# Rose-STL-Lab/spherical-dyffusion

Hardware: AMD Instinct MI355X
Metric: forecast-steps/sec (180x360, 63ch), 25-member ensemble DYffusion sampling, whole job (higher is better)
Workload: dtype f32 tensors; every GEMM-class kernel (1x1 convs, fused MLP, Legendre analysis/synthesis, dhconv) as 3-pass split-f16 MFMA with f32 accumulation; FFT / norms / pointwise in f32 (statistics f64)

## Files before the change

### include/sdy_amd.h

```cpp
#ifndef SDY_AMD_H
#define SDY_AMD_H

#include <stddef.h>
#include <stdint.h>

#ifdef __cplusplus
extern "C" {
#endif
#pragma GCC visibility push(default)

#define SDY_OK 0
#define SDY_ERR_ARG (-1)
#define SDY_ERR_UNSUPPORTED (-2)
#define SDY_ERR_ALIGN (-3)
#define SDY_ERR_WORKSPACE (-4)
#define SDY_ERR_NAME (-5)
#define SDY_ERR_SHAPE (-6)
#define SDY_ERR_STATE (-7)

#define SDY_GRID_EQUIANGULAR 0
#define SDY_GRID_LEGENDRE_GAUSS 1

int sdy_version(void);
const char* sdy_error_string(int code);
// ... 3 lines not shown

typedef struct sdy_sht_plan sdy_sht_plan;

int sdy_sht_tables_host(int nlat, int nlon, int lmax, int mmax, int grid, double* pct, double* w, double* theta);

int sdy_sht_plan_create(int nlat, int nlon, int lmax, int mmax, int grid, sdy_sht_plan** out);
int sdy_sht_plan_create_ex(int nlat, int nlon, int lmax, int mmax, int grid, int gemm_mode, sdy_sht_plan** out);
void sdy_sht_plan_destroy(sdy_sht_plan* plan);
int sdy_sht_plan_dims(const sdy_sht_plan* plan, int dims[6]);
int sdy_sht_plan_kernels(const sdy_sht_plan* plan, int out[2]);
size_t sdy_sht_workspace_floats(const sdy_sht_plan* plan, int B, int C);

int sdy_sht_forward(const sdy_sht_plan* plan, const float* x, float* out_c64, int B, int C, float* ws,
                    size_t ws_floats, void* stream);
int sdy_sht_inverse(const sdy_sht_plan* plan, const float* in_c64, float* y, int B, int C, float* ws,
                    size_t ws_floats, void* stream);

int sdy_rfft_lon(const sdy_sht_plan* plan, const float* x, const float* a, const float* d, float* xn_out,
                 float* Xf, int B, int C, void* stream);
int sdy_legendre_fwd(const sdy_sht_plan* plan, const float* Xf, float* Cs, int B, int C, void* stream);
int sdy_legendre_inv(const sdy_sht_plan* plan, const float* Cs, float* Yf, int B, int C, void* stream);
int sdy_irfft_lon(const sdy_sht_plan* plan, const float* Yf, const float* bias, float* y, int B, int C,
                  void* stream);
int sdy_irfft_lon_act(const sdy_sht_plan* plan, const float* Yf, const float* bias, float* zt, long zt_bstride, double* part,
                      int B, int C, void* stream);
int sdy_instnorm_from_partials(const double* part, int K, int B, int C, int HW, const float* gamma, const float* beta,
                               float eps, float* a, float* d, void* stream);
int sdy_gelu_stats(const float* y, long y_bstride, float* out, long out_bstride, int out_tiled, double* stats, int B, int C,
                   int HW, void* stream);
int sdy_affine_copy_stats(const float* x, long x_bstride, const float* a, const float* d, float* out, long out_bstride,
                          double* stats, int C, int HW, const unsigned char* rows, int n_rows, int src_row0, void* stream);

int sdy_dhconv_pack_weight(const float* w_host, int Ci, int Co, int L, float* w_packed_dev, void* stream);
int sdy_dhconv(const float* Cs_in, const float* w_packed, float* Cs_out, int L, int mtr, int B, int Ci, int Co,
               void* stream);
size_t sdy_dhconv_h3_pack_bytes(int Ci, int Co, int L);
int sdy_dhconv_h3_pack_weight(const float* w_host, int Ci, int Co, int L, void* packed_dev, float* scale);
int sdy_dhconv_h3(const float* Cs_in, const void* packed, float scale, float* Cs_out, int L, int mtr, int B, int Ci,
                  int Co, void* stream);

int sdy_dhconv_frag_supported(int Ci, int Co);
size_t sdy_dhconv_frag_pack_bytes(int L);
int sdy_dhconv_frag_pack(const float* w_host, int L, void* packed_dev, float* scale);
int sdy_dhconv_frag(const float* Cs_in, const void* packed, float scale, float* Cs_out, int L, int mtr, int B,
                    void* stream);

// ... 437 lines not shown
```

### spherical-dyffusion_amd/_lib.py

```python
from __future__ import annotations

import ctypes as C
import os

_HERE = os.path.dirname(os.path.abspath(__file__))
LIB_PATH = os.environ.get("SDY_AMD_LIB") or os.path.join(_HERE, "libsdy_amd.so")

SDY_GRID = {"equiangular": 0, "legendre-gauss": 1}


class SdyError(RuntimeError):
    pass


class SdyConvArgs(C.Structure):
    _fields_ = [
        ("x", C.c_void_p), ("x_bstride", C.c_long),
        ("wt", C.c_void_p), ("ldw", C.c_int),
        ("out", C.c_void_p), ("out_bstride", C.c_long),
        ("B", C.c_int), ("Cin", C.c_int), ("Cout", C.c_int), ("HW", C.c_int),
        ("pa", C.c_void_p), ("pd", C.c_void_p),
        ("bias", C.c_void_p),
        ("add", C.c_void_p), ("add_bstride", C.c_long),
        ("add_mode", C.c_int),
# ... 319 lines not shown
               SdyMemberSumArgs, SdyMemberStatsArgs, SdySpectrumArgs, SdyVariabilityArgs, SdyVariabilityMapsArgs,
               SdyVariabilityStatsArgs, SdyRegionSeriesArgs, SdyRankHistArgs)

SIGNATURES = {
    "sdy_version": (C.c_int, []),
    "sdy_error_string": (C.c_char_p, [C.c_int]),
    "sdy_abi_check": (C.c_int, [C.POINTER(C.c_size_t), C.c_int]),
    "sdy_abi_sizes": (C.c_int, [C.POINTER(C.c_size_t), C.c_int]),
    "sdy_sht_tables_host": (C.c_int, [C.c_int, C.c_int, C.c_int, C.c_int, C.c_int, C.c_void_p, C.c_void_p, C.c_void_p]),
    "sdy_sht_plan_create": (C.c_int, [C.c_int, C.c_int, C.c_int, C.c_int, C.c_int, C.POINTER(C.c_void_p)]),
    "sdy_sht_plan_create_ex": (C.c_int, [C.c_int, C.c_int, C.c_int, C.c_int, C.c_int, C.c_int, C.POINTER(C.c_void_p)]),
    "sdy_sht_plan_destroy": (None, [C.c_void_p]),
    "sdy_sht_plan_dims": (C.c_int, [C.c_void_p, C.POINTER(C.c_int * 6)]),
    "sdy_sht_plan_kernels": (C.c_int, [C.c_void_p, C.POINTER(C.c_int * 2)]),
    "sdy_sht_workspace_floats": (C.c_size_t, [C.c_void_p, C.c_int, C.c_int]),
    "sdy_sht_forward": (C.c_int, [C.c_void_p, C.c_void_p, C.c_void_p, C.c_int, C.c_int, C.c_void_p, C.c_size_t, C.c_void_p]),
    "sdy_sht_inverse": (C.c_int, [C.c_void_p, C.c_void_p, C.c_void_p, C.c_int, C.c_int, C.c_void_p, C.c_size_t, C.c_void_p]),
    "sdy_rfft_lon": (C.c_int, [C.c_void_p, C.c_void_p, C.c_void_p, C.c_void_p, C.c_void_p, C.c_void_p, C.c_int, C.c_int, C.c_void_p]),
    "sdy_legendre_fwd": (C.c_int, [C.c_void_p, C.c_void_p, C.c_void_p, C.c_int, C.c_int, C.c_void_p]),
    "sdy_legendre_inv": (C.c_int, [C.c_void_p, C.c_void_p, C.c_void_p, C.c_int, C.c_int, C.c_void_p]),
    "sdy_irfft_lon": (C.c_int, [C.c_void_p, C.c_void_p, C.c_void_p, C.c_void_p, C.c_int, C.c_int, C.c_void_p]),
    "sdy_irfft_lon_act": (C.c_int, [C.c_void_p, C.c_void_p, C.c_void_p, C.c_void_p, C.c_long, C.c_void_p, C.c_int, C.c_int,
                                    C.c_void_p]),
    "sdy_instnorm_from_partials": (C.c_int, [C.c_void_p, C.c_int, C.c_int, C.c_int, C.c_int, C.c_void_p, C.c_void_p, C.c_float,
                                             C.c_void_p, C.c_void_p, C.c_void_p]),
    "sdy_gelu_stats": (C.c_int, [C.c_void_p, C.c_long, C.c_void_p, C.c_long, C.c_int, C.c_void_p, C.c_int, C.c_int, C.c_int,
                                 C.c_void_p]),
    "sdy_affine_copy_stats": (C.c_int, [C.c_void_p, C.c_long, C.c_void_p, C.c_void_p, C.c_void_p, C.c_long, C.c_void_p, C.c_int,
                                        C.c_int, C.c_void_p, C.c_int, C.c_int, C.c_void_p]),
    "sdy_dhconv_pack_weight": (C.c_int, [C.c_void_p, C.c_int, C.c_int, C.c_int, C.c_void_p, C.c_void_p]),
    "sdy_dhconv": (C.c_int, [C.c_void_p, C.c_void_p, C.c_void_p, C.c_int, C.c_int, C.c_int, C.c_int, C.c_int, C.c_void_p]),
    "sdy_dhconv_h3_pack_bytes": (C.c_size_t, [C.c_int, C.c_int, C.c_int]),
    "sdy_dhconv_h3_pack_weight": (C.c_int, [C.c_void_p, C.c_int, C.c_int, C.c_int, C.c_void_p, C.POINTER(C.c_float)]),
    "sdy_dhconv_h3": (C.c_int, [C.c_void_p, C.c_void_p, C.c_float, C.c_void_p, C.c_int, C.c_int, C.c_int, C.c_int, C.c_int,
                                C.c_void_p]),
    "sdy_dhconv_frag_supported": (C.c_int, [C.c_int, C.c_int]),
    "sdy_dhconv_frag_pack_bytes": (C.c_size_t, [C.c_int]),
    "sdy_dhconv_frag_pack": (C.c_int, [C.c_void_p, C.c_int, C.c_void_p, C.POINTER(C.c_float)]),
    "sdy_dhconv_frag": (C.c_int, [C.c_void_p, C.c_void_p, C.c_float, C.c_void_p, C.c_int, C.c_int, C.c_int, C.c_void_p]),
    "sdy_instnorm_coeffs": (C.c_int, [C.c_void_p, C.c_int, C.c_int, C.c_int, C.c_void_p, C.c_void_p, C.c_void_p, C.c_long,
                                      C.c_float, C.c_void_p, C.c_void_p, C.c_void_p]),
    "sdy_conv1x1": (C.c_int, [C.POINTER(SdyConvArgs), C.c_void_p]),
    "sdy_ensemble_metrics": (C.c_int, [C.c_void_p, C.c_void_p, C.c_void_p, C.c_int, C.c_long, C.c_int, C.c_int, C.c_void_p,
                                       C.c_void_p]),
    "sdy_instnorm_from_stats": (C.c_int, [C.c_void_p, C.c_int, C.c_int, C.c_int, C.c_void_p, C.c_void_p, C.c_void_p,
                                          C.c_long, C.c_float, C.c_void_p, C.c_void_p, C.c_void_p]),
# ... 155 lines not shown
```

### spherical-dyffusion_amd/csrc/capi.hip

```cpp
#include <cmath>
#include <cstdio>
#include <cstdlib>
#include <cstring>
#include <mutex>
#include <string>
#include <vector>

#include "common.h"
#include "fft.h"
#include "pointwise.h"

static inline int round_up(int v, int m) { return (v + m - 1) / m * m; }
static inline size_t round_up_sz(size_t v, size_t m) { return (v + m - 1) / m * m; }

template <class F>
static float h3_pack_host(std::vector<_Float16>& buf, int nb, int rows, int K, int rows_pad, int Kpad, F value) {
  float mx = 0.f;
  for (int b = 0; b < nb; ++b)
    for (int r = 0; r < rows; ++r)
      for (int k = 0; k < K; ++k) mx = std::fmax(mx, std::fabs(value(b, r, k)));
  const float s = sdy_h3_scale(mx);
  const size_t plane = (size_t)nb * rows_pad * Kpad;
  buf.assign(2 * plane, (_Float16)0.0f);
  for (int b = 0; b < nb; ++b)
// ... 449 lines not shown

extern "C" int sdy_affine_copy_stats(const float* x, long x_bstride, const float* a, const float* d, float* out,
                                     long out_bstride, double* stats, int C, int HW, const unsigned char* rows, int n_rows,
                                     int src_row0, void* stream) {
  if (!x || !out || !rows || (a == nullptr) != (d == nullptr) || C <= 0 || HW <= 0 || n_rows <= 0 || n_rows > SDY_MAP_MAX ||
      x_bstride < 0 || out_bstride < 0)
    return SDY_ERR_ARG;
  if ((HW & 3) || (x_bstride & 3) || (out_bstride & 3) || !fft_aligned16(x) || !fft_aligned16(out) || !fft_aligned16(stats))
    return SDY_ERR_ALIGN;
  return sdy_affine_copy_stats_launch(x, x_bstride, a, d, out, out_bstride, stats, C, HW, rows, n_rows, (hipStream_t)stream,
                                      src_row0 >= 0 ? src_row0 : -1);
}

extern "C" int sdy_irfft_lon_act(const sdy_sht_plan* p, const float* Yf, const float* bias, float* zt, long zt_bstride,
                                 double* part, int B, int C, void* stream) {
  if (!p || !Yf || !zt || !part || B <= 0 || C <= 0 || zt_bstride < 0) return SDY_ERR_ARG;
  if (C % 4 != 0 || (zt_bstride & 3) || !fft_aligned16(Yf) || !fft_aligned16(zt) || !fft_aligned16(part)) return SDY_ERR_ALIGN;
  if (!(p->fft.fft360 && p->fft.n == 180) || C % 16 != 0) return SDY_ERR_UNSUPPORTED;
  if (!tiled_stride_ok(zt_bstride, C, p->nlat * p->nlon)) return SDY_ERR_ARG;
  return sdy_fft360_launch_inv(p->fft, Yf, bias, nullptr, B, C, p->nlat, p->mtr, 0, nullptr, (hipStream_t)stream, zt, zt_bstride,
                               part);
}

static inline int h3_mpad(int Cout) { return Cout > 128 ? round_up(Cout, 256) : 128; }
static inline int h3_kpad(int Cin) { return round_up(Cin, 64); }

extern "C" size_t sdy_h3_pack_bytes(int Cout, int Cin) {
  if (Cout <= 0 || Cin <= 0) return 0;
  return (size_t)2 * h3_mpad(Cout) * h3_kpad(Cin) * sizeof(_Float16);
}

extern "C" int sdy_h3_pack_weight(const float* w, int Cout, int Cin, void* packed_dev, float* scale) {
  if (!w || !packed_dev || !scale || Cout <= 0 || Cin <= 0) return SDY_ERR_ARG;
  std::vector<_Float16> buf;
  *scale = h3_pack_host(buf, 1, Cout, Cin, h3_mpad(Cout), h3_kpad(Cin),
                        [&](int, int o, int i) { return w[(size_t)o * Cin + i]; });
  SDY_HIP_TRY(hipMemcpy(packed_dev, buf.data(), buf.size() * sizeof(_Float16), hipMemcpyHostToDevice));
  return SDY_OK;
}

extern "C" int sdy_conv1x1(const sdy_conv_args* a, void* stream) {
  if (!a || !a->x || (!a->wt && !a->w_h3 && !a->w_frag) || !a->out) return SDY_ERR_ARG;
  if (a->B <= 0 || a->Cin <= 0 || a->Cout <= 0 || a->HW <= 0) return SDY_ERR_ARG;
  if (!a->w_h3 && a->ldw < a->Cout) return SDY_ERR_ARG;
  if ((a->pa == nullptr) != (a->pd == nullptr)) return SDY_ERR_ARG;
  if (a->add_mode != 0 && !a->add) return SDY_ERR_ARG;
// ... 962 lines not shown
```

### spherical-dyffusion_amd/csrc/fft.h

```cpp
#pragma once
#include <hip/hip_runtime.h>

struct SdyFftDesc {
  int n;
  int S;
  int nstages;
  int radices[10];
  const float* tw;
  const float* pw;
  int guard_f16;
  int fft360;
};


int sdy_fft_launch_fwd(const SdyFftDesc& f, const float* x, const float* a, const float* d, float* xn_out, float* Xf,
                       int B, int C, int K, int mtr, int ilv, const int* mcut, hipStream_t stream,
                       const unsigned char* x_rows = nullptr, int x_mod = 0);
int sdy_fft_launch_inv(const SdyFftDesc& f, const float* Yf, const float* bias, float* y, int B, int C, int K, int mtr,
                       int ilv, const int* mcut, hipStream_t stream);

int sdy_fft360_launch_fwd(const SdyFftDesc& f, const float* x, const float* a, const float* d, float* xn_out, float* Xf,
                          int B, int C, int K, int mtr, int ilv, const int* mcut, hipStream_t stream,
                          const unsigned char* x_rows = nullptr, int x_mod = 0);
int sdy_fft360_launch_inv(const SdyFftDesc& f, const float* Yf, const float* bias, float* y, int B, int C, int K,
                          int mtr, int ilv, const int* mcut, hipStream_t stream, float* zt = nullptr, long zt_bs = 0,
                          double* part = nullptr);
```

### spherical-dyffusion_amd/csrc/fft360.hip

```cpp
#include "common.h"
#include "fft.h"

namespace {

typedef float c2 __attribute__((ext_vector_type(2)));

constexpr int NH = 180;
constexpr int NLON = 360;
constexpr int ROWS = 16;
constexpr int NT = 256;
constexpr int P = 200;
constexpr int Q4 = NLON / 4;
constexpr int MIT = 3;
#ifndef SDY_FFT_MINB_F
#define SDY_FFT_MINB_F 4
#endif
#ifndef SDY_FFT_MINB_I
#define SDY_FFT_MINB_I 4
#endif
#ifndef SDY_FFT_KPW
#define SDY_FFT_KPW 1
#endif
constexpr int MINB_F = SDY_FFT_MINB_F, MINB_I = SDY_FFT_MINB_I;

template <int SG>
__device__ __forceinline__ c2 mul_i(c2 a) {
  return SG > 0 ? c2{-a.y, a.x} : c2{a.y, -a.x};
}
__device__ __forceinline__ c2 cmul(c2 a, c2 w) { return a.xx * w + a.yy * c2{-w.y, w.x}; }
__device__ __forceinline__ c2 cmul_conj(c2 a, c2 w) { return a.xx * c2{w.x, -w.y} + a.yy * c2{w.y, w.x}; }

template <int SG>
__device__ __forceinline__ void dft3(c2& v0, c2& v1, c2& v2) {
  const float sn = 0.86602540378443864676f;
  const c2 a = v1 + v2, b = v1 - v2;
  const c2 m = v0 - 0.5f * a;
  const c2 t = mul_i<SG>(sn * b);
  v0 = v0 + a;
  v1 = m + t;
  v2 = m - t;
}
template <int SG>
__device__ __forceinline__ void dft4(c2& v0, c2& v1, c2& v2, c2& v3) {
  const c2 t0 = v0 + v2, t1 = v0 - v2, t2 = v1 + v3, t3 = mul_i<SG>(v1 - v3);
  v0 = t0 + t2;
  v1 = t1 + t3;
// ... 84 lines not shown
    for (int k2 = 0; k2 < 15; ++k2) dst[12 * k2] = u[pfa_slot<3, 5>(k2)];
    if (NYQ_COPY && L.t == 0) dst[NH] = u[pfa_slot<3, 5>(0)];
  }
  __builtin_amdgcn_wave_barrier();
}
template <int SG>
__device__ __forceinline__ void pass_a_tail(const Lane& L, c2* v, const c2* TW) {
  pfa<3, 4, SG>(v);
  c2* dst = L.row + L.t;
  const c2* tw = TW + L.t;
  dst[0] = v[pfa_slot<3, 4>(0)];
#pragma unroll
  for (int k1 = 1; k1 < 12; ++k1) {
    const c2 y = v[pfa_slot<3, 4>(k1)];
    dst[15 * k1] = SG < 0 ? cmul(y, tw[16 * k1]) : cmul_conj(y, tw[16 * k1]);
  }
}

constexpr int TAIL = Q4 - 64;

#ifndef SDY_FFT_GROUP
#define SDY_FFT_GROUP 4
#endif
struct WgId {
  int x, y, z;
};
__device__ __forceinline__ WgId wg_id(int nx, int ny) {
  const unsigned total = gridDim.x, L = blockIdx.x;
  const unsigned xcd = L % 8u, slot = L / 8u;
  const unsigned id = xcd * (total / 8u) + min(xcd, total % 8u) + slot;
  WgId w;
#if SDY_FFT_GROUP > 0
  if (nx % SDY_FFT_GROUP == 0) {
    const unsigned G = SDY_FFT_GROUP;
    w.x = (int)(G * ((id / (G * ny)) % ((unsigned)nx / G)) + id % G);
    w.y = (int)((id / G) % (unsigned)ny);
    w.z = (int)(id / ((unsigned)nx * ny));
    return w;
  }
#endif
  w.x = id % nx;
  w.y = (id / nx) % ny;
  w.z = id / (nx * ny);
  return w;
}

template <int KPW>
__global__ __launch_bounds__(NT, MINB_F) void rfft360_kernel(const SdyFftDesc f, const float* __restrict__ x,
                                                           const float* __restrict__ pa, const float* __restrict__ pd,
                                                           float* __restrict__ xn_out, float* __restrict__ Xf, int B,
                                                           int C, int K, int mtr, int ilv,
                                                           const int* __restrict__ mcut, const SdyImgMap xmap,
                                                           unsigned* flags, unsigned* head, int x_mod) {
  __shared__ __attribute__((aligned(16))) c2 Z[ROWS * P];
  __shared__ c2 TW[TWN];
  __shared__ c2 AD[ROWS];
  const Lane L = lane_roles(Z);
  const WgId id = wg_id(C / ROWS, (K + KPW - 1) / KPW);
  const int c0 = id.x * ROWS, b = id.z;
  const int bx = sdy_img(xmap, b);
  const int k_begin = id.y * KPW, k_end = min(K, k_begin + KPW);

  fill_twiddles(f, TW);
  if (threadIdx.x < ROWS) {
    const int s = threadIdx.x, ch = c0 + 4 * (s & 3) + (s >> 2);
    AD[s] = pa ? c2{pa[bx * C + ch], pd[bx * C + ch]} : c2{1.0f, 0.0f};
  }

  const int bsrc = x_mod > 0 ? bx % x_mod : bx;
  const float* xw = x + (((long)bsrc * C + c0 + L.wave) * K) * NLON + 4 * L.lane;
  float* xnw = xn_out ? xn_out + (((long)bx * C + c0 + L.wave) * K) * NLON + 4 * L.lane : nullptr;
  const long rstride = 4L * K * NLON;
  c2* zw = Z + 4 * L.wave * P + 2 * L.lane;
  const bool tail = L.lane < TAIL;

  const int c4 = threadIdx.x & 3, mg = threadIdx.x >> 2;
  const float scale = 6.28318530717958647692f / (float)NLON;
  c2 W[MIT];
#pragma unroll
  for (int it = 0; it < MIT; ++it) {
    const c2 w = reinterpret_cast<const c2*>(f.pw)[min(mg + 64 * it, NH)];
    W[it] = c2{w.y, -w.x} * (0.5f * scale);
  }
  const c2* za = Z + c4 * P + mg;
  const c2* zn01 = Z + c4 * P + (NH - 64 - mg);
  const c2* zn2 = Z + c4 * P + max(NH - 128 - mg, 0);
  const long mstride = (long)K * B * 2 * C;
  const int re_off = (ilv ? 2 * c0 : c0) + 4 * c4, im_off = ilv ? 16 : C;
  const long tile_base = (long)((b * (C / ROWS) + id.x) >> 1) * K * 64 + (id.x & 1) * 32 + 4 * c4;

  float amax = 0.0f;
  f32x4 regs[8];
  auto gload = [&](int k) {
#pragma unroll
    for (int r = 0; r < 4; ++r) {
      const float* src = xw + r * rstride + (long)k * NLON;
      regs[2 * r] = *reinterpret_cast<const f32x4*>(src);
      if (tail) regs[2 * r + 1] = *reinterpret_cast<const f32x4*>(src + 256);
    }
  };
  gload(k_begin);
  __syncthreads();

  for (int k = k_begin; k < k_end; ++k) {
#pragma unroll
    for (int r = 0; r < 4; ++r) {
      const c2 ad = AD[4 * L.wave + r];
      const f32x4 v0 = regs[2 * r] * ad.x + ad.y, v1 = regs[2 * r + 1] * ad.x + ad.y;
      if (xnw) {
        float* dst = xnw + r * rstride + (long)k * NLON;
        *reinterpret_cast<f32x4*>(dst) = v0;
        if (tail) *reinterpret_cast<f32x4*>(dst + 256) = v1;
      }
      *reinterpret_cast<f32x4*>(zw + r * P) = v0;
      if (tail) *reinterpret_cast<f32x4*>(zw + r * P + 128) = v1;
    }
    if (k + 1 < k_end) gload(k + 1);
    __builtin_amdgcn_wave_barrier();

    if (L.t < 15) {
      c2 v[12];
      const c2* src = L.row + L.t;
#pragma unroll
      for (int bb = 0; bb < 12; ++bb) v[bb] = src[15 * bb];
      pass_a_tail<-1>(L, v, TW);
    }
    pass_b<-1, true>(L);
    __syncthreads();

    float* Xk = ilv == 2 ? Xf + tile_base + (long)k * 64 : Xf + ((long)k * B + b) * 2 * C + re_off;
    const int mlive = mcut ? min(mtr, mcut[k]) : mtr;
#pragma unroll
    for (int it = 0; it < MIT; ++it) {
      const int m = mg + 64 * it;
      if (m < mlive) {
        f32x4 vr, vi;
#pragma unroll
        for (int j = 0; j < 4; ++j) {
          const c2 A = za[64 * it + 4 * j * P];
          const c2 Bv = it < 2 ? zn01[64 * (1 - it) + 4 * j * P] : zn2[4 * j * P];
          const c2 S = c2{A.x + Bv.x, A.y - Bv.y}, D = c2{A.x - Bv.x, A.y + Bv.y};
          const c2 X = (0.5f * scale) * S + cmul(D, W[it]);
          vr[j] = X.x;
          vi[j] = X.y;
          amax = __builtin_fmaxf(amax, __builtin_fmaxf(__builtin_fabsf(X.x), __builtin_fabsf(X.y)));
        }
        float* o = Xk + (long)m * mstride;
        SDY_STREAM_STORE(o, vr);
        SDY_STREAM_STORE(o + im_off, vi);
      }
    }
    __syncthreads();
  }
  sdy_flag_range(flags, amax * (2.0f * SDY_ACT_SX), head);
}

template <int KPW>
__global__ __launch_bounds__(NT, MINB_I) void irfft360_kernel(const SdyFftDesc f, const float* __restrict__ Yf,
                                                            const float* __restrict__ bias, float* __restrict__ y, int B,
                                                            int C, int K, int mtr, int ilv,
                                                            const int* __restrict__ mcut, float* __restrict__ zt,
                                                            long zt_bs, double* __restrict__ part) {
  __shared__ __attribute__((aligned(16))) c2 Z[ROWS * P];
  __shared__ c2 TW[TWN];
  __shared__ c2 PW[NH];
  __shared__ float BS[ROWS];
  const Lane L = lane_roles(Z);
  const WgId id = wg_id(C / ROWS, (K + KPW - 1) / KPW);
  const int c0 = id.x * ROWS, b = id.z;
  const int k_begin = id.y * KPW, k_end = min(K, k_begin + KPW);

  fill_twiddles(f, TW);
  if (threadIdx.x < NH) {
    const c2 w = reinterpret_cast<const c2*>(f.pw)[threadIdx.x];
    PW[threadIdx.x] = c2{w.x, -w.y};
  }
  if (threadIdx.x < ROWS) {
    const int s = threadIdx.x;
    BS[s] = bias ? bias[c0 + 4 * (s & 3) + (s >> 2)] : 0.0f;
  }

  const int c4 = threadIdx.x & 3, mg = threadIdx.x >> 2;
  const long mstride = (long)K * B * 2 * C;
  const int re_off = (ilv ? 2 * c0 : c0) + 4 * c4, im_off = ilv ? 16 : C;
  const long tile_base = (long)((b * (C / ROWS) + id.x) >> 1) * K * 64 + (id.x & 1) * 32 + 4 * c4;
  f32x4 rr[MIT], ri[MIT];
  auto gload = [&](int k) {
    const float* Yk = ilv == 2 ? Yf + tile_base + (long)k * 64 : Yf + ((long)k * B + b) * 2 * C + re_off;
    const int mlive = mcut ? min(mtr, mcut[k]) : mtr;
#pragma unroll
    for (int it = 0; it < MIT; ++it) {
      const int m = mg + 64 * it;
      f32x4 vr = {0.f, 0.f, 0.f, 0.f}, vi = {0.f, 0.f, 0.f, 0.f};
      if (m < mlive) {
        const float* o = Yk + (long)m * mstride;
        vr = *reinterpret_cast<const f32x4*>(o);
        vi = *reinterpret_cast<const f32x4*>(o + im_off);
      }
      if (m == 0 || m == NH) vi = f32x4{0.f, 0.f, 0.f, 0.f};
      rr[it] = vr;
      ri[it] = vi;
    }
  };

  float* yw = y + (((long)b * C + c0 + L.wave) * K) * NLON + 4 * L.lane;
  const long rstride = 4L * K * NLON;
  const c2* zw = Z + 4 * L.wave * P + 2 * L.lane;
  const bool tail = L.lane < TAIL;
  c2* zs = Z + c4 * P + mg;

  gload(k_begin);
  for (int k = k_begin; k < k_end; ++k) {
#pragma unroll
    for (int it = 0; it < MIT; ++it) {
      if (mg + 64 * it <= NH) {
#pragma unroll
        for (int j = 0; j < 4; ++j) zs[4 * j * P + 64 * it] = c2{rr[it][j], ri[it][j]};
      }
    }
    __syncthreads();
    if (k + 1 < k_end) gload(k + 1);

    if (L.t < 15) {
      c2 v[12];
      const c2* lo = L.row + L.t;
      const c2* hi = L.row + (15 - L.t);
      const c2* pw = PW + L.t;
#pragma unroll
      for (int bb = 0; bb < 12; ++bb) {
        const c2 A = lo[15 * bb], Bv = hi[15 * (11 - bb)], w = pw[15 * bb];
        const c2 S = c2{A.x + Bv.x, A.y - Bv.y}, Dm = c2{A.x - Bv.x, A.y + Bv.y};
        const c2 D = cmul(Dm, w);
        v[bb] = c2{S.x - D.y, S.y + D.x};
      }
      __builtin_amdgcn_wave_barrier();
      pass_a_tail<+1>(L, v, TW);
    }
    pass_b<+1, false>(L);

    if (zt) {
      float* ztb = zt + (long)b * zt_bs;
      const int px0 = k * NLON + 4 * L.lane, px1 = px0 + 256;
#pragma unroll
      for (int r = 0; r < 4; ++r) {
        const float bs = BS[4 * L.wave + r];
        const int ch = c0 + L.wave + 4 * r;
        f32x4 v = *reinterpret_cast<const f32x4*>(zw + r * P) + bs;
        v = f32x4{gelu_erf(v.x), gelu_erf(v.y), gelu_erf(v.z), gelu_erf(v.w)};
        SDY_STREAM_STORE(ztb + (long)(px0 >> 6) * (C * 64) + ch * 64 + (px0 & 63), v);
        float qs = sdy_quad_sum(v), qs2 = sdy_quad_sumsq(v);
        if (tail) {
          f32x4 u = *reinterpret_cast<const f32x4*>(zw + r * P + 128) + bs;
          u = f32x4{gelu_erf(u.x), gelu_erf(u.y), gelu_erf(u.z), gelu_erf(u.w)};
          SDY_STREAM_STORE(ztb + (long)(px1 >> 6) * (C * 64) + ch * 64 + (px1 & 63), u);
          qs += sdy_quad_sum(u);
          qs2 += sdy_quad_sumsq(u);
        }
        double ds = (double)row16_sum(qs), ds2 = (double)row16_sum(qs2);
        ds += __shfl_xor(ds, 16, 64);
        ds2 += __shfl_xor(ds2, 16, 64);
        ds += __shfl_xor(ds, 32, 64);
        ds2 += __shfl_xor(ds2, 32, 64);
        if (L.lane == 0) {
          double* slot = part + (((long)b * K + k) * C + ch) * 2;
          slot[0] = ds;
          slot[1] = ds2;
        }
      }
    } else {
#pragma unroll
    for (int r = 0; r < 4; ++r) {
      const float bs = BS[4 * L.wave + r];
      float* dst = yw + r * rstride + (long)k * NLON;
      SDY_STREAM_STORE(dst, *reinterpret_cast<const f32x4*>(zw + r * P) + bs);
      if (tail) SDY_STREAM_STORE(dst + 256, *reinterpret_cast<const f32x4*>(zw + r * P + 128) + bs);
    }
    }
    __syncthreads();
  }
}

}

int sdy_fft360_launch_fwd(const SdyFftDesc& f, const float* x, const float* a, const float* d, float* xn_out, float* Xf,
                          int B, int C, int K, int mtr, int ilv, const int* mcut, hipStream_t stream,
                          const unsigned char* x_rows, int x_mod) {
  if (f.n != NH || C % ROWS != 0 || mtr > NH + 1 || (long)ROWS * K * NLON >= (1L << 31)) return SDY_ERR_UNSUPPORTED;
  if (ilv == 2 && (C % (2 * ROWS) != 0 || ROWS != 16)) return SDY_ERR_UNSUPPORTED;
  constexpr int KPW = SDY_FFT_KPW;
  SdyImgMap xmap;
  SDY_TRY(sdy_img_map_fill(xmap, x_rows, B));
  dim3 grid((C / ROWS) * ((K + KPW - 1) / KPW) * B);
  unsigned *flags = nullptr, *head = nullptr;
  if (f.guard_f16) {
    SDY_TRY(sdy_flags_ptr(&flags));
    SDY_TRY(sdy_headroom_ptr(SDY_RANGE_LEG_ANALYSIS, &head));
  }
  hipLaunchKernelGGL((rfft360_kernel<KPW>), grid, dim3(NT), 0, stream, f, x, a, d, xn_out, Xf, B, C, K, mtr, ilv, mcut, xmap,
                     flags, head, x_mod);
  return sdy_launch_status();
}

int sdy_fft360_launch_inv(const SdyFftDesc& f, const float* Yf, const float* bias, float* y, int B, int C, int K,
                          int mtr, int ilv, const int* mcut, hipStream_t stream, float* zt, long zt_bs, double* part) {
  if (f.n != NH || C % ROWS != 0 || mtr > NH + 1 || (long)ROWS * K * NLON >= (1L << 31)) return SDY_ERR_UNSUPPORTED;
  if (ilv == 2 && (C % (2 * ROWS) != 0 || ROWS != 16)) return SDY_ERR_UNSUPPORTED;
  if ((zt == nullptr) != (part == nullptr) || (!zt && !y)) return SDY_ERR_ARG;
  constexpr int KPW = SDY_FFT_KPW;
  dim3 grid((C / ROWS) * ((K + KPW - 1) / KPW) * B);
  hipLaunchKernelGGL((irfft360_kernel<KPW>), grid, dim3(NT), 0, stream, f, Yf, bias, y, B, C, K, mtr, ilv, mcut, zt, zt_bs, part);
  return sdy_launch_status();
}
```

### spherical-dyffusion_amd/csrc/pointwise.hip

```cpp
#include <cmath>
#include <atomic>
#include <mutex>
#include <vector>
#include "common.h"
#include "pointwise.h"

namespace {

inline bool al16(const void* p) { return ((uintptr_t)p & 15) == 0; }

__global__ __launch_bounds__(256) void instnorm_coeffs_kernel(const float* __restrict__ x, int C, int HW,
                                                               const float* __restrict__ gamma,
                                                               const float* __restrict__ beta,
                                                               const float* __restrict__ ss, long ss_stride, float eps,
                                                               float* __restrict__ a_out, float* __restrict__ d_out,
                                                               unsigned* __restrict__ flags) {
  const int c = blockIdx.x, b = blockIdx.y;
  const float* px = x + ((long)b * C + c) * HW;
  double s = 0.0, s2 = 0.0;
  const int n4 = HW >> 2;
  const f32x4* p4 = reinterpret_cast<const f32x4*>(px);
  for (int i = threadIdx.x; i < n4; i += 256) {
    const f32x4 v = p4[i];
    s += (double)v.x + (double)v.y + (double)v.z + (double)v.w;
// ... 46 lines not shown
  const int i = blockIdx.x * 256 + threadIdx.x;
  if (i >= BC) return;
  const int b = i / C, c = i - b * C;
  const double S = stats[2 * (long)i], S2 = stats[2 * (long)i + 1];
  stats[2 * (long)i] = 0.0;
  stats[2 * (long)i + 1] = 0.0;
  if (flags && !(fabs(S) <= 1.7e308 && S2 <= 1.7e308)) atomicOr(flags, (unsigned)SDY_FLAG_NONFINITE);
  const double mean = S / HW;
  double var = S2 / HW - mean * mean;
  if (var < 0.0) var = 0.0;
  const float rstd = (float)(1.0 / sqrt(var + (double)eps));
  float a = gamma[c] * rstd;
  float d = beta[c] - (float)mean * a;
  if (ss) {
    const float sc = ss[(long)b * ss_stride + c] + 1.0f;
    const float sh_ = ss[(long)b * ss_stride + C + c];
    a = a * sc;
    d = d * sc + sh_;
  }
  a_out[i] = a;
  d_out[i] = d;
}

__global__ __launch_bounds__(256) void instnorm_from_partials_kernel(const double* __restrict__ part, int K, int BC, int C, int HW,
                                                                      const float* __restrict__ gamma,
                                                                      const float* __restrict__ beta, float eps,
                                                                      float* __restrict__ a_out, float* __restrict__ d_out,
                                                                      unsigned* __restrict__ flags) {
  const int i = blockIdx.x * 256 + threadIdx.x;
  if (i >= BC) return;
  const int b = i / C, c = i - b * C;
  const double* q = part + ((long)b * K * C + c) * 2;
  constexpr int G = 20;
  double S = 0.0, S2 = 0.0;
  int k = 0;
  for (; k + G <= K; k += G) {
    double v[G], w[G];
#pragma unroll
    for (int j = 0; j < G; ++j) {
      v[j] = q[(long)(k + j) * C * 2];
      w[j] = q[(long)(k + j) * C * 2 + 1];
    }
#pragma unroll
    for (int j = 0; j < G; ++j) {
      S += v[j];
      S2 += w[j];
    }
  }
  for (; k < K; ++k) {
    S += q[(long)k * C * 2];
    S2 += q[(long)k * C * 2 + 1];
  }
  if (flags && !(fabs(S) <= 1.7e308 && S2 <= 1.7e308)) atomicOr(flags, (unsigned)SDY_FLAG_NONFINITE);
  const double mean = S / HW;
  double var = S2 / HW - mean * mean;
  if (var < 0.0) var = 0.0;
  const float rstd = (float)(1.0 / sqrt(var + (double)eps));
  const float a = gamma[c] * rstd;
  a_out[i] = a;
  d_out[i] = beta[c] - (float)mean * a;
}

__global__ __launch_bounds__(256) void affine_copy_stats_kernel(const float* __restrict__ x, long x_bs,
                                                                 const float* __restrict__ a, const float* __restrict__ d,
                                                                 float* __restrict__ out, long out_bs,
                                                                 double* __restrict__ stats, int C, int HW,
                                                                 const SdyImgMap rows, int src_row0) {
  const int c = blockIdx.x, b = sdy_img(rows, blockIdx.y), bs = src_row0 >= 0 ? src_row0 + (int)blockIdx.y : b;
  const f32x4* p4 = reinterpret_cast<const f32x4*>(x + (long)bs * x_bs + (long)c * HW);
  f32x4* o4 = reinterpret_cast<f32x4*>(out + (long)b * out_bs + (long)c * HW);
  const float av = a ? a[b * C + c] : 1.0f, dv = a ? d[b * C + c] : 0.0f;
  double s = 0.0, s2 = 0.0;
  const int n4 = HW >> 2;
  for (int i = threadIdx.x; i < n4; i += 256) {
    const f32x4 r = p4[i];
// ... 815 lines not shown
  SDY_TRY(sdy_flags_ptr(&flags));
  hipLaunchKernelGGL(instnorm_coeffs_kernel, dim3(C, B), dim3(256), 0, stream, x, C, HW, gamma, beta, ss, ss_stride,
                     eps, a, d, flags);
  return sdy_launch_status();
}

extern "C" int sdy_instnorm_from_stats(double* stats, int B, int C, int HW, const float* gamma, const float* beta,
                                       const float* ss, long ss_stride, float eps, float* a, float* d, void* stream) {
  if (!stats || !gamma || !beta || !a || !d || B <= 0 || C <= 0 || HW <= 0) return SDY_ERR_ARG;
  const int BC = B * C;
  unsigned* flags = nullptr;
  SDY_TRY(sdy_flags_ptr(&flags));
  hipLaunchKernelGGL(instnorm_from_stats_kernel, dim3((BC + 255) / 256), dim3(256), 0, (hipStream_t)stream, stats, BC, C, HW,
                     gamma, beta, ss, ss_stride, eps, a, d, flags);
  return sdy_launch_status();
}

int sdy_instnorm_from_partials_launch(const double* part, int K, int B, int C, int HW, const float* gamma, const float* beta,
                                      float eps, float* a, float* d, hipStream_t stream) {
  if (!part || !gamma || !beta || !a || !d || K <= 0 || B <= 0 || C <= 0 || HW <= 0) return SDY_ERR_ARG;
  const int BC = B * C;
  unsigned* flags = nullptr;
  SDY_TRY(sdy_flags_ptr(&flags));
  hipLaunchKernelGGL(instnorm_from_partials_kernel, dim3((BC + 255) / 256), dim3(256), 0, stream, part, K, BC, C, HW, gamma, beta, eps,
                     a, d, flags);
  return sdy_launch_status();
}

int sdy_gelu_stats_launch(const float* y, long y_bs, float* out, long out_bs, int out_tiled, double* stats, int B, int C,
                          int HW, hipStream_t stream) {
  if (!y || !out || B <= 0 || C <= 0 || HW <= 0) return SDY_ERR_ARG;
  if ((HW & 3) || (y_bs & 3) || (out_bs & 3)) return SDY_ERR_ALIGN;
  hipLaunchKernelGGL(gelu_stats_kernel, dim3(C, B), dim3(256), 0, stream, y, y_bs, out, out_bs, out_tiled, stats, C, HW);
  return sdy_launch_status();
}

int sdy_affine_copy_stats_launch(const float* x, long x_bs, const float* a, const float* d, float* out, long out_bs,
                                 double* stats, int C, int HW, const unsigned char* rows, int n_rows, hipStream_t stream,
                                 int src_row0) {
  if (!x || (a == nullptr) != (d == nullptr) || !out || !rows || C <= 0 || HW <= 0 || n_rows <= 0) return SDY_ERR_ARG;
  if ((HW & 3) || (x_bs & 3) || (out_bs & 3)) return SDY_ERR_ALIGN;
  SdyImgMap m;
  SDY_TRY(sdy_img_map_fill(m, rows, n_rows));
  hipLaunchKernelGGL(affine_copy_stats_kernel, dim3(C, n_rows), dim3(256), 0, stream, x, x_bs, a, d, out, out_bs, stats, C, HW, m,
                     src_row0);
  return sdy_launch_status();
}

// ... 114 lines not shown
```

Measured before the change: 164.7.

## Add multi-ring runs to FFT360 kernels and rework instnorm partial reduction

The forward rfft360 kernel now handles several latitude rings per workgroup, using either a strided or a contiguous walk. It prefetches the next ring's loads while the current one is in the FFT passes, and picks the run length at launch from CU count and grid fill. The inverse kernel now issues its first global load before filling twiddles, and gets zero-masking on register-resident data (it defaults to one ring per workgroup). instnorm_from_partials is rewritten so each block reduces 8 channels over rings using coalesced double2 loads staged in shared memory, replacing one strided thread per channel. Fewer workgroups with more rings each can reduce occupancy, and debug timestamp hooks plus new C API entry points are also added.

Result: no change. 164.6 (-0.1%).

```diff
diff --git a/include/sdy_amd.h b/include/sdy_amd.h
--- a/include/sdy_amd.h
+++ b/include/sdy_amd.h
@@ -49,6 +49,11 @@
 int sdy_legendre_inv(const sdy_sht_plan* plan, const float* Cs, float* Yf, int B, int C, void* stream);
 int sdy_irfft_lon(const sdy_sht_plan* plan, const float* Yf, const float* bias, float* y, int B, int C,
                   void* stream);
+int sdy_rfft360_lon(const sdy_sht_plan* plan, const float* x, const float* a, const float* d, float* xn_out, float* Xf,
+                    int B, int C, int layout, const int* mcut, const unsigned char* x_rows, int x_mod, int ring_run,
+                    void* stream);
+int sdy_irfft360_lon(const sdy_sht_plan* plan, const float* Yf, const float* bias, float* y, float* zt, long zt_bstride,
+                     double* part, int B, int C, int layout, const int* mcut, int ring_run, void* stream);
 int sdy_irfft_lon_act(const sdy_sht_plan* plan, const float* Yf, const float* bias, float* zt, long zt_bstride, double* part,
                       int B, int C, void* stream);
 int sdy_instnorm_from_partials(const double* part, int K, int B, int C, int HW, const float* gamma, const float* beta,
diff --git a/spherical-dyffusion_amd/_lib.py b/spherical-dyffusion_amd/_lib.py
--- a/spherical-dyffusion_amd/_lib.py
+++ b/spherical-dyffusion_amd/_lib.py
@@ -365,6 +365,10 @@
     "sdy_irfft_lon": (C.c_int, [C.c_void_p, C.c_void_p, C.c_void_p, C.c_void_p, C.c_int, C.c_int, C.c_void_p]),
     "sdy_irfft_lon_act": (C.c_int, [C.c_void_p, C.c_void_p, C.c_void_p, C.c_void_p, C.c_long, C.c_void_p, C.c_int, C.c_int,
                                     C.c_void_p]),
+    "sdy_rfft360_lon": (C.c_int, [C.c_void_p, C.c_void_p, C.c_void_p, C.c_void_p, C.c_void_p, C.c_void_p, C.c_int, C.c_int,
+                                  C.c_int, C.c_void_p, C.c_void_p, C.c_int, C.c_int, C.c_void_p]),
+    "sdy_irfft360_lon": (C.c_int, [C.c_void_p, C.c_void_p, C.c_void_p, C.c_void_p, C.c_void_p, C.c_long, C.c_void_p, C.c_int,
+                                   C.c_int, C.c_int, C.c_void_p, C.c_int, C.c_void_p]),
     "sdy_instnorm_from_partials": (C.c_int, [C.c_void_p, C.c_int, C.c_int, C.c_int, C.c_int, C.c_void_p, C.c_void_p, C.c_float,
                                              C.c_void_p, C.c_void_p, C.c_void_p]),
     "sdy_gelu_stats": (C.c_int, [C.c_void_p, C.c_long, C.c_void_p, C.c_long, C.c_int, C.c_void_p, C.c_int, C.c_int, C.c_int,
diff --git a/spherical-dyffusion_amd/csrc/capi.hip b/spherical-dyffusion_amd/csrc/capi.hip
--- a/spherical-dyffusion_amd/csrc/capi.hip
+++ b/spherical-dyffusion_amd/csrc/capi.hip
@@ -495,6 +495,35 @@
                                part);
 }
 
+static int fft360_ex_check(const sdy_sht_plan* p, int B, int C, int layout, int ring_run) {
+  if (!p || B <= 0 || C <= 0 || layout < 0 || layout > 2) return SDY_ERR_ARG;
+  if (ring_run != 0 && ring_run != 1 && ring_run != 2 && ring_run != 4 && ring_run != 8) return SDY_ERR_ARG;
+  if (C % 4 != 0) return SDY_ERR_ALIGN;
+  if (!(p->fft.fft360 && p->fft.n == 180) || C % 16 != 0 || (layout == 2 && C % 32 != 0)) return SDY_ERR_UNSUPPORTED;
+  return SDY_OK;
+}
+
+extern "C" int sdy_rfft360_lon(const sdy_sht_plan* p, const float* x, const float* a, const float* d, float* xn_out, float* Xf,
+                               int B, int C, int layout, const int* mcut, const unsigned char* x_rows, int x_mod,
+                               int ring_run, void* stream) {
+  if (!x || !Xf || (a == nullptr) != (d == nullptr) || x_mod < 0 || (x_rows && B > SDY_MAP_MAX)) return SDY_ERR_ARG;
+  SDY_TRY(fft360_ex_check(p, B, C, layout, ring_run));
+  if (!fft_aligned16(x) || !fft_aligned16(xn_out) || !fft_aligned16(Xf)) return SDY_ERR_ALIGN;
+  return sdy_fft360_launch_fwd(p->fft, x, a, d, xn_out, Xf, B, C, p->nlat, p->mtr, layout, mcut, (hipStream_t)stream, x_rows,
+                               x_mod, ring_run);
+}
+
+extern "C" int sdy_irfft360_lon(const sdy_sht_plan* p, const float* Yf, const float* bias, float* y, float* zt, long zt_bstride,
+                                double* part, int B, int C, int layout, const int* mcut, int ring_run, void* stream) {
+  if (!Yf || (y == nullptr) == (zt == nullptr) || (zt == nullptr) != (part == nullptr) || zt_bstride < 0) return SDY_ERR_ARG;
+  SDY_TRY(fft360_ex_check(p, B, C, layout, ring_run));
+  if ((zt_bstride & 3) || !fft_aligned16(Yf) || !fft_aligned16(y) || !fft_aligned16(zt) || !fft_aligned16(part))
+    return SDY_ERR_ALIGN;
+  if (zt && !tiled_stride_ok(zt_bstride, C, p->nlat * p->nlon)) return SDY_ERR_ARG;
+  return sdy_fft360_launch_inv(p->fft, Yf, bias, y, B, C, p->nlat, p->mtr, layout, mcut, (hipStream_t)stream, zt, zt_bstride,
+                               part, ring_run);
+}
+
 static inline int h3_mpad(int Cout) { return Cout > 128 ? round_up(Cout, 256) : 128; }
 static inline int h3_kpad(int Cin) { return round_up(Cin, 64); }
 
diff --git a/spherical-dyffusion_amd/csrc/fft.h b/spherical-dyffusion_amd/csrc/fft.h
--- a/spherical-dyffusion_amd/csrc/fft.h
+++ b/spherical-dyffusion_amd/csrc/fft.h
@@ -21,7 +21,7 @@
 
 int sdy_fft360_launch_fwd(const SdyFftDesc& f, const float* x, const float* a, const float* d, float* xn_out, float* Xf,
                           int B, int C, int K, int mtr, int ilv, const int* mcut, hipStream_t stream,
-                          const unsigned char* x_rows = nullptr, int x_mod = 0);
+                          const unsigned char* x_rows = nullptr, int x_mod = 0, int ring_run = 0);
 int sdy_fft360_launch_inv(const SdyFftDesc& f, const float* Yf, const float* bias, float* y, int B, int C, int K,
                           int mtr, int ilv, const int* mcut, hipStream_t stream, float* zt = nullptr, long zt_bs = 0,
-                          double* part = nullptr);
+                          double* part = nullptr, int ring_run = 0);
diff --git a/spherical-dyffusion_amd/csrc/fft360.hip b/spherical-dyffusion_amd/csrc/fft360.hip
--- a/spherical-dyffusion_amd/csrc/fft360.hip
+++ b/spherical-dyffusion_amd/csrc/fft360.hip
@@ -1,3 +1,5 @@
+#include <cstdlib>
+
 #include "common.h"
 #include "fft.h"
 
@@ -18,10 +20,24 @@
 #ifndef SDY_FFT_MINB_I
 #define SDY_FFT_MINB_I 4
 #endif
-#ifndef SDY_FFT_KPW
-#define SDY_FFT_KPW 1
+#ifndef SDY_FFT_RUN_MAX_F
+#define SDY_FFT_RUN_MAX_F 4
+#endif
+#ifndef SDY_FFT_RUN_MAX_I
+#define SDY_FFT_RUN_MAX_I 1
 #endif
 constexpr int MINB_F = SDY_FFT_MINB_F, MINB_I = SDY_FFT_MINB_I;
+
+__device__ __forceinline__ void retire_loads() {
+  __builtin_amdgcn_s_waitcnt(0x0F70);
+  __builtin_amdgcn_sched_barrier(0);
+}
+
+#define SDY_FFT_STAMP(r, i)                                                                            \
+  do {                                                                                                 \
+    if (SDY_STAMPS_ON && stamps && blockIdx.x == (gridDim.x >> 1) && threadIdx.x == 0 && (r) < 8)      \
+      stamps[(r) * 8 + (i)] = __builtin_amdgcn_s_memtime();                                            \
+  } while (0)
 
 template <int SG>
 __device__ __forceinline__ c2 mul_i(c2 a) {
@@ -152,6 +168,20 @@
 #ifndef SDY_FFT_GROUP
 #define SDY_FFT_GROUP 4
 #endif
+#ifndef SDY_FFT_RING_STRIDE
+#define SDY_FFT_RING_STRIDE 1
+#endif
+struct RingWalk {
+  int k0, step, n;
+};
+template <int RUN>
+__device__ __forceinline__ RingWalk ring_walk(int y, int K) {
+  if (RUN == 1) return RingWalk{y, 1, 1};
+  const int ny = (K + RUN - 1) / RUN;
+  if (SDY_FFT_RING_STRIDE) return RingWalk{y, ny, (K - 1 - y) / ny + 1};
+  return RingWalk{y * RUN, 1, min(RUN, K - y * RUN)};
+}
+
 struct WgId {
   int x, y, z;
 };
@@ -175,21 +205,23 @@
   return w;
 }
 
-template <int KPW>
+template <int RUN>
 __global__ __launch_bounds__(NT, MINB_F) void rfft360_kernel(const SdyFftDesc f, const float* __restrict__ x,
                                                            const float* __restrict__ pa, const float* __restrict__ pd,
                                                            float* __restrict__ xn_out, float* __restrict__ Xf, int B,
                                                            int C, int K, int mtr, int ilv,
                                                            const int* __restrict__ mcut, const SdyImgMap xmap,
-                                                           unsigned* flags, unsigned* head, int x_mod) {
+                                                           unsigned* flags, unsigned* head, int x_mod,
+                                                           unsigned long long* stamps) {
   __shared__ __attribute__((aligned(16))) c2 Z[ROWS * P];
   __shared__ c2 TW[TWN];
   __shared__ c2 AD[ROWS];
   const Lane L = lane_roles(Z);
-  const WgId id = wg_id(C / ROWS, (K + KPW - 1) / KPW);
+  const WgId id = wg_id(C / ROWS, (K + RUN - 1) / RUN);
   const int c0 = id.x * ROWS, b = id.z;
   const int bx = sdy_img(xmap, b);
-  const int k_begin = id.y * KPW, k_end = min(K, k_begin + KPW);
+  const RingWalk rw = ring_walk<RUN>(id.y, K);
+  SDY_FFT_STAMP(0, 0);
 
   fill_twiddles(f, TW);
   if (threadIdx.x < ROWS) {
@@ -229,10 +261,13 @@
       if (tail) regs[2 * r + 1] = *reinterpret_cast<const f32x4*>(src + 256);
     }
   };
-  gload(k_begin);
+  gload(rw.k0);
   __syncthreads();
-
-  for (int k = k_begin; k < k_end; ++k) {
+  if (RUN > 1 || SDY_STAMPS_ON) retire_loads();
+  SDY_FFT_STAMP(0, 1);
+
+  for (int j = 0, k = rw.k0; j < rw.n; ++j, k += rw.step) {
+    if (j > 0) SDY_FFT_STAMP(j, 0);
 #pragma unroll
     for (int r = 0; r < 4; ++r) {
       const c2 ad = AD[4 * L.wave + r];
@@ -245,8 +280,9 @@
       *reinterpret_cast<f32x4*>(zw + r * P) = v0;
       if (tail) *reinterpret_cast<f32x4*>(zw + r * P + 128) = v1;
     }
-    if (k + 1 < k_end) gload(k + 1);
+    if (j + 1 < rw.n) gload(k + rw.step);
     __builtin_amdgcn_wave_barrier();
+    SDY_FFT_STAMP(j, 2);
 
     if (L.t < 15) {
       c2 v[12];
@@ -255,8 +291,12 @@
       for (int bb = 0; bb < 12; ++bb) v[bb] = src[15 * bb];
       pass_a_tail<-1>(L, v, TW);
     }
+    SDY_FFT_STAMP(j, 3);
     pass_b<-1, true>(L);
     __syncthreads();
+    SDY_FFT_STAMP(j, 4);
+    if (RUN > 1) retire_loads();
+    SDY_FFT_STAMP(j, 5);
 
     float* Xk = ilv == 2 ? Xf + tile_base + (long)k * 64 : Xf + ((long)k * B + b) * 2 * C + re_off;
     const int mlive = mcut ? min(mtr, mcut[k]) : mtr;
@@ -280,56 +320,47 @@
         SDY_STREAM_STORE(o + im_off, vi);
       }
     }
+    SDY_FFT_STAMP(j, 6);
     __syncthreads();
+    SDY_FFT_STAMP(j, 7);
   }
   sdy_flag_range(flags, amax * (2.0f * SDY_ACT_SX), head);
 }
 
-template <int KPW>
+template <int RUN>
 __global__ __launch_bounds__(NT, MINB_I) void irfft360_kernel(const SdyFftDesc f, const float* __restrict__ Yf,
                                                             const float* __restrict__ bias, float* __restrict__ y, int B,
                                                             int C, int K, int mtr, int ilv,
                                                             const int* __restrict__ mcut, float* __restrict__ zt,
-                                                            long zt_bs, double* __restrict__ part) {
+                                                            long zt_bs, double* __restrict__ part,
+                                                            unsigned long long* stamps) {
   __shared__ __attribute__((aligned(16))) c2 Z[ROWS * P];
   __shared__ c2 TW[TWN];
   __shared__ c2 PW[NH];
   __shared__ float BS[ROWS];
   const Lane L = lane_roles(Z);
-  const WgId id = wg_id(C / ROWS, (K + KPW - 1) / KPW);
+  const WgId id = wg_id(C / ROWS, (K + RUN - 1) / RUN);
   const int c0 = id.x * ROWS, b = id.z;
-  const int k_begin = id.y * KPW, k_end = min(K, k_begin + KPW);
-
-  fill_twiddles(f, TW);
-  if (threadIdx.x < NH) {
-    const c2 w = reinterpret_cast<const c2*>(f.pw)[threadIdx.x];
-    PW[threadIdx.x] = c2{w.x, -w.y};
-  }
-  if (threadIdx.x < ROWS) {
-    const int s = threadIdx.x;
-    BS[s] = bias ? bias[c0 + 4 * (s & 3) + (s >> 2)] : 0.0f;
-  }
+  const RingWalk rw = ring_walk<RUN>(id.y, K);
+  SDY_FFT_STAMP(0, 0);
 
   const int c4 = threadIdx.x & 3, mg = threadIdx.x >> 2;
   const long mstride = (long)K * B * 2 * C;
   const int re_off = (ilv ? 2 * c0 : c0) + 4 * c4, im_off = ilv ? 16 : C;
   const long tile_base = (long)((b * (C / ROWS) + id.x) >> 1) * K * 64 + (id.x & 1) * 32 + 4 * c4;
-  f32x4 rr[MIT], ri[MIT];
+  f32x4 rr[MIT] = {}, ri[MIT] = {};
+  int mlive_nxt = 0;
   auto gload = [&](int k) {
     const float* Yk = ilv == 2 ? Yf + tile_base + (long)k * 64 : Yf + ((long)k * B + b) * 2 * C + re_off;
-    const int mlive = mcut ? min(mtr, mcut[k]) : mtr;
+    mlive_nxt = mcut ? min(mtr, mcut[k]) : mtr;
 #pragma unroll
     for (int it = 0; it < MIT; ++it) {
       const int m = mg + 64 * it;
-      f32x4 vr = {0.f, 0.f, 0.f, 0.f}, vi = {0.f, 0.f, 0.f, 0.f};
-      if (m < mlive) {
+      if (m < mlive_nxt) {
         const float* o = Yk + (long)m * mstride;
-        vr = *reinterpret_cast<const f32x4*>(o);
-        vi = *reinterpret_cast<const f32x4*>(o + im_off);
+        rr[it] = *reinterpret_cast<const f32x4*>(o);
+        ri[it] = *reinterpret_cast<const f32x4*>(o + im_off);
       }
-      if (m == 0 || m == NH) vi = f32x4{0.f, 0.f, 0.f, 0.f};
-      rr[it] = vr;
-      ri[it] = vi;
     }
   };
 
@@ -339,17 +370,33 @@
   const bool tail = L.lane < TAIL;
   c2* zs = Z + c4 * P + mg;
 
-  gload(k_begin);
-  for (int k = k_begin; k < k_end; ++k) {
+  gload(rw.k0);
+  fill_twiddles(f, TW);
+  if (threadIdx.x < NH) {
+    const c2 w = reinterpret_cast<const c2*>(f.pw)[threadIdx.x];
+    PW[threadIdx.x] = c2{w.x, -w.y};
+  }
+  if (threadIdx.x < ROWS) {
+    const int s = threadIdx.x;
+    BS[s] = bias ? bias[c0 + 4 * (s & 3) + (s >> 2)] : 0.0f;
+  }
+  if (RUN > 1 || SDY_STAMPS_ON) retire_loads();
+  SDY_FFT_STAMP(0, 1);
+  for (int j = 0, k = rw.k0; j < rw.n; ++j, k += rw.step) {
+    if (j > 0) SDY_FFT_STAMP(j, 0);
+    const int mlive = mlive_nxt;
 #pragma unroll
     for (int it = 0; it < MIT; ++it) {
-      if (mg + 64 * it <= NH) {
-#pragma unroll
-        for (int j = 0; j < 4; ++j) zs[4 * j * P + 64 * it] = c2{rr[it][j], ri[it][j]};
+      const int m = mg + 64 * it;
+      if (m <= NH) {
+        const bool re_live = m < mlive, im_live = re_live && m != 0 && m != NH;
+#pragma unroll
+        for (int j = 0; j < 4; ++j) zs[4 * j * P + 64 * it] = c2{re_live ? rr[it][j] : 0.0f, im_live ? ri[it][j] : 0.0f};
       }
     }
     __syncthreads();
-    if (k + 1 < k_end) gload(k + 1);
+    SDY_FFT_STAMP(j, 2);
+    if (j + 1 < rw.n) gload(k + rw.step);
 
     if (L.t < 15) {
       c2 v[12];
@@ -366,7 +413,11 @@
       __builtin_amdgcn_wave_barrier();
       pass_a_tail<+1>(L, v, TW);
     }
+    SDY_FFT_STAMP(j, 3);
     pass_b<+1, false>(L);
+    SDY_FFT_STAMP(j, 4);
+    if (RUN > 1) retire_loads();
+    SDY_FFT_STAMP(j, 5);
 
     if (zt) {
       float* ztb = zt + (long)b * zt_bs;
@@ -406,38 +457,106 @@
       if (tail) SDY_STREAM_STORE(dst + 256, *reinterpret_cast<const f32x4*>(zw + r * P + 128) + bs);
     }
     }
+    SDY_FFT_STAMP(j, 6);
     __syncthreads();
-  }
-}
-
+    SDY_FFT_STAMP(j, 7);
+  }
+}
+
+}
+
+#if SDY_STAMPS_ON
+static unsigned long long* g_fstamps = nullptr;
+SDY_DEBUG_EXPORT int sdy_fft360_debug_stamps(unsigned long long* host192) {
+  if (!g_fstamps || !host192) return SDY_ERR_STATE;
+  SDY_HIP_TRY(hipDeviceSynchronize());
+  SDY_HIP_TRY(hipMemcpy(host192, g_fstamps, 192 * sizeof(unsigned long long), hipMemcpyDeviceToHost));
+  return SDY_OK;
+}
+#endif
+static int fft_stamps(int which, unsigned long long** stamps) {
+  *stamps = nullptr;
+#if SDY_STAMPS_ON
+  if (std::getenv("SDY_FFT_STAMPS")) {
+    if (!g_fstamps) {
+      SDY_HIP_TRY(hipMalloc(&g_fstamps, 192 * sizeof(unsigned long long)));
+      SDY_HIP_TRY(hipMemset(g_fstamps, 0, 192 * sizeof(unsigned long long)));
+    }
+    *stamps = g_fstamps + 64 * which;
+  }
+#endif
+  return SDY_OK;
+}
+
+constexpr int RUN_FILL = 8;
+static int pick_run(int forced, int run_max, int nx, int K, int B, int* run) {
+  if (forced) {
+    if (forced != 1 && forced != 2 && forced != 4 && forced != 8) return SDY_ERR_ARG;
+    *run = forced;
+    return SDY_OK;
+  }
+  int n_cu = 0;
+  SDY_TRY(sdy_cu_count(&n_cu));
+  int r = run_max;
+  if (r == 1) {
+    *run = 1;
+    return SDY_OK;
+  }
+  while (r > 1 && (long)nx * ((K + r - 1) / r) * B < (long)RUN_FILL * 4 * n_cu) r >>= 1;
+  *run = r;
+  return SDY_OK;
 }
 
 int sdy_fft360_launch_fwd(const SdyFftDesc& f, const float* x, const float* a, const float* d, float* xn_out, float* Xf,
                           int B, int C, int K, int mtr, int ilv, const int* mcut, hipStream_t stream,
-                          const unsigned char* x_rows, int x_mod) {
+                          const unsigned char* x_rows, int x_mod, int ring_run) {
   if (f.n != NH || C % ROWS != 0 || mtr > NH + 1 || (long)ROWS * K * NLON >= (1L << 31)) return SDY_ERR_UNSUPPORTED;
   if (ilv == 2 && (C % (2 * ROWS) != 0 || ROWS != 16)) return SDY_ERR_UNSUPPORTED;
-  constexpr int KPW = SDY_FFT_KPW;
+  int run = 1;
+  SDY_TRY(pick_run(ring_run, SDY_FFT_RUN_MAX_F, C / ROWS, K, B, &run));
   SdyImgMap xmap;
   SDY_TRY(sdy_img_map_fill(xmap, x_rows, B));
-  dim3 grid((C / ROWS) * ((K + KPW - 1) / KPW) * B);
+  dim3 grid((C / ROWS) * ((K + run - 1) / run) * B);
   unsigned *flags = nullptr, *head = nullptr;
   if (f.guard_f16) {
     SDY_TRY(sdy_flags_ptr(&flags));
     SDY_TRY(sdy_headroom_ptr(SDY_RANGE_LEG_ANALYSIS, &head));
   }
-  hipLaunchKernelGGL((rfft360_kernel<KPW>), grid, dim3(NT), 0, stream, f, x, a, d, xn_out, Xf, B, C, K, mtr, ilv, mcut, xmap,
-                     flags, head, x_mod);
+  unsigned long long* stamps = nullptr;
+  SDY_TRY(fft_stamps(0, &stamps));
+#define SDY_FFT_FWD(R)                                                                                                      \
+  hipLaunchKernelGGL((rfft360_kernel<R>), grid, dim3(NT), 0, stream, f, x, a, d, xn_out, Xf, B, C, K, mtr, ilv, mcut, xmap, \
+                     flags, head, x_mod, stamps)
+  switch (run) {
+    case 1: SDY_FFT_FWD(1); break;
+    case 2: SDY_FFT_FWD(2); break;
+    case 4: SDY_FFT_FWD(4); break;
+    default: SDY_FFT_FWD(8); break;
+  }
+#undef SDY_FFT_FWD
   return sdy_launch_status();
 }
 
 int sdy_fft360_launch_inv(const SdyFftDesc& f, const float* Yf, const float* bias, float* y, int B, int C, int K,
-                          int mtr, int ilv, const int* mcut, hipStream_t stream, float* zt, long zt_bs, double* part) {
+                          int mtr, int ilv, const int* mcut, hipStream_t stream, float* zt, long zt_bs, double* part,
+                          int ring_run) {
   if (f.n != NH || C % ROWS != 0 || mtr > NH + 1 || (long)ROWS * K * NLON >= (1L << 31)) return SDY_ERR_UNSUPPORTED;
   if (ilv == 2 && (C % (2 * ROWS) != 0 || ROWS != 16)) return SDY_ERR_UNSUPPORTED;
   if ((zt == nullptr) != (part == nullptr) || (!zt && !y)) return SDY_ERR_ARG;
-  constexpr int KPW = SDY_FFT_KPW;
-  dim3 grid((C / ROWS) * ((K + KPW - 1) / KPW) * B);
-  hipLaunchKernelGGL((irfft360_kernel<KPW>), grid, dim3(NT), 0, stream, f, Yf, bias, y, B, C, K, mtr, ilv, mcut, zt, zt_bs, part);
+  int run = 1;
+  SDY_TRY(pick_run(ring_run, SDY_FFT_RUN_MAX_I, C / ROWS, K, B, &run));
+  dim3 grid((C / ROWS) * ((K + run - 1) / run) * B);
+  unsigned long long* stamps = nullptr;
+  SDY_TRY(fft_stamps(zt ? 2 : 1, &stamps));
+#define SDY_FFT_INV(R)                                                                                                        \
+  hipLaunchKernelGGL((irfft360_kernel<R>), grid, dim3(NT), 0, stream, f, Yf, bias, y, B, C, K, mtr, ilv, mcut, zt, zt_bs, part, \
+                     stamps)
+  switch (run) {
+    case 1: SDY_FFT_INV(1); break;
+    case 2: SDY_FFT_INV(2); break;
+    case 4: SDY_FFT_INV(4); break;
+    default: SDY_FFT_INV(8); break;
+  }
+#undef SDY_FFT_INV
   return sdy_launch_status();
 }
diff --git a/spherical-dyffusion_amd/csrc/pointwise.hip b/spherical-dyffusion_amd/csrc/pointwise.hip
--- a/spherical-dyffusion_amd/csrc/pointwise.hip
+++ b/spherical-dyffusion_amd/csrc/pointwise.hip
@@ -92,35 +92,40 @@
   d_out[i] = d;
 }
 
+constexpr int PART_SLOTS = 8, PART_RINGS = 128;
 __global__ __launch_bounds__(256) void instnorm_from_partials_kernel(const double* __restrict__ part, int K, int BC, int C, int HW,
                                                                       const float* __restrict__ gamma,
                                                                       const float* __restrict__ beta, float eps,
                                                                       float* __restrict__ a_out, float* __restrict__ d_out,
                                                                       unsigned* __restrict__ flags) {
-  const int i = blockIdx.x * 256 + threadIdx.x;
-  if (i >= BC) return;
+  __shared__ double2 sh[PART_RINGS * PART_SLOTS];
+  const double2* part2 = reinterpret_cast<const double2*>(part);
+  const int i0 = blockIdx.x * PART_SLOTS, n = min(PART_SLOTS, BC - i0);
+  const int i = i0 + (int)threadIdx.x;
+  const int s = threadIdx.x % PART_SLOTS, is = i0 + s;
+  const int bs = is / C, cs = is - bs * C;
+  double S = 0.0, S2 = 0.0;
+  for (int k0 = 0; k0 < K; k0 += PART_RINGS) {
+    const int kn = min(PART_RINGS, K - k0);
+    if (s < n) {
+#pragma unroll
+      for (int j = 0; j < PART_RINGS * PART_SLOTS / 256; ++j) {
+        const int kk = (int)threadIdx.x / PART_SLOTS + j * (256 / PART_SLOTS);
+        if (kk < kn) sh[kk * PART_SLOTS + s] = part2[((long)bs * K + k0 + kk) * C + cs];
+      }
+    }
+    __syncthreads();
+    if ((int)threadIdx.x < n) {
+      for (int kk = 0; kk < kn; ++kk) {
+        const double2 v = sh[kk * PART_SLOTS + threadIdx.x];
+        S += v.x;
+        S2 += v.y;
+      }
+    }
+    __syncthreads();
+  }
+  if ((int)threadIdx.x >= n) return;
   const int b = i / C, c = i - b * C;
-  const double* q = part + ((long)b * K * C + c) * 2;
-  constexpr int G = 20;
-  double S = 0.0, S2 = 0.0;
-  int k = 0;
-  for (; k + G <= K; k += G) {
-    double v[G], w[G];
-#pragma unroll
-    for (int j = 0; j < G; ++j) {
-      v[j] = q[(long)(k + j) * C * 2];
-      w[j] = q[(long)(k + j) * C * 2 + 1];
-    }
-#pragma unroll
-    for (int j = 0; j < G; ++j) {
-      S += v[j];
-      S2 += w[j];
-    }
-  }
-  for (; k < K; ++k) {
-    S += q[(long)k * C * 2];
-    S2 += q[(long)k * C * 2 + 1];
-  }
   if (flags && !(fabs(S) <= 1.7e308 && S2 <= 1.7e308)) atomicOr(flags, (unsigned)SDY_FLAG_NONFINITE);
   const double mean = S / HW;
   double var = S2 / HW - mean * mean;
@@ -982,8 +987,8 @@
   const int BC = B * C;
   unsigned* flags = nullptr;
   SDY_TRY(sdy_flags_ptr(&flags));
-  hipLaunchKernelGGL(instnorm_from_partials_kernel, dim3((BC + 255) / 256), dim3(256), 0, stream, part, K, BC, C, HW, gamma, beta, eps,
-                     a, d, flags);
+  hipLaunchKernelGGL(instnorm_from_partials_kernel, dim3((BC + PART_SLOTS - 1) / PART_SLOTS), dim3(256), 0, stream, part, K, BC, C,
+                     HW, gamma, beta, eps, a, d, flags);
   return sdy_launch_status();
 }
 
```
